# duowuyms/MANSY_ImmersiveVideoStreaming

Hardware: AMD Instinct MI355X
Metric: viewport-trajectories/sec (VP train) (higher is better)
Workload: dtype f32; 1 GPU; VP Transformer train step (fwd+loss+bwd+AdamW), B=4096/GPU synthetic torus-walk trajectories len 21 (hist 10 + cur 1 + pred 10), d=512, 8 heads, 2+2 layers, dropout on, fp32 MFMA, decoder recurrence as two half-batches on two streams; two_stream=True, global_batch=4096, parallelism=dp1

## Files before the change

### include/mansy_hip.h

```cpp
#ifndef MANSY_HIP_H
#define MANSY_HIP_H
#include <stddef.h>
#include <stdint.h>

#ifdef __cplusplus
extern "C" {
#endif

const char* mansy_last_error(void);
int mansy_abi_version(void);

#define MANSY_PREC_F32 0
#define MANSY_PREC_BF16 1
#define MANSY_PREC_BF16X3 3
#define MANSY_PREC_BF16X6 6

typedef int (*mansy_bn_sync_fn)(int which, void* user);

typedef struct mansy_vp_config {
  int B, S, T;
  int d_model, n_head, d_ff;
  int n_enc, n_dec;
  int in_ch;
  int has_bias;
// ... 149 lines not shown
int mansy_identifier_train_step(const float* const* params, float* const* grads, float* flat_p, float* flat_g, float* flat_m,
                                float* flat_v, long long n_flat, const float* obs, const int* idx ,
                                int B, float lr, float weight_decay, int step, float* loss_out, void* workspace, int max_batch,
                                void* xg_ctx ,
                                const float* adam_bias , int precision, void* stream);
int mansy_identifier_relabel(const float* const* params, const float* obs, float* rew, float* id_rew, int B, float lamb,
                             void* workspace, int max_batch, int precision, void* stream);
int mansy_gae_returns(const float* rew, const float* v_s, const float* v_next, const unsigned char* done, int T, int N, double gamma,
                      double gae_lambda, int rew_norm, double* rms, double* scratch, float* returns, float* adv, void* stream);
int mansy_ppo_minibatch_step(const float* const* params, float* const* grads, float* flat_p, float* flat_g, float* flat_m,
                             float* flat_v, long long n_flat, const float* obs_all, const int* idx, const int* act_all,
                             const float* adv_all, const float* logp_old_all, const float* v_old_all, const float* ret_all, int mb,
                             float eps_clip, float vf_coef, float ent_coef, int norm_adv, int value_clip, float dual_clip,
                             float max_grad_norm, float lr, float weight_decay, int step, long long tail_from, int tail_step, float* stats,
                             void* workspace, int max_batch, int chain_in, const int* next_idx, int next_mb, void* xg_ctx, const float* adam_bias,
                             int precision, void* stream);
int mansy_bc_step(const float* const* params, float* const* grads, float* flat_p, float* flat_g, float* flat_m, float* flat_v,
                  long long n_flat, long long n_update, const float* obs, const int* act, int B, float ent_coef, float lr,
                  float weight_decay, int step, float* stats, void* workspace, int max_batch, int precision, void* stream);

#define MANSY_CLIP_SCRATCH_DOUBLES 64
int mansy_clip_grad_adam(float* flat_p, float* flat_g, float* flat_m, float* flat_v, long long n_flat, float max_grad_norm, float lr,
                         float weight_decay, int step, long long tail_from, int tail_step, double* scratch, int have_sumsq,
                         const float* adam_bias , void* stream);

int mansy_ppo_dp_tail(const float* const* params, float* flat_p, float* flat_g, float* flat_m, float* flat_v, long long n_flat,
                      float max_grad_norm, float lr, float weight_decay, int step, double* scratch, int have_sumsq, const float* obs_all,
                      const float* adv_all, const int* next_idx, int next_mb, float* next_flat_g, const float* adam_bias , void* workspace,
                      int max_batch, int precision, void* stream);

typedef struct mansy_comm_id { unsigned char bytes[128]; } mansy_comm_id;
int mansy_comm_unique_id(mansy_comm_id* out);
int mansy_comm_create(const mansy_comm_id* id, int world, int rank, void** comm_out);
int mansy_comm_destroy(void* comm);
int mansy_allreduce_avg_f32(void* comm, float* buf , long long n, void* stream);
int mansy_allreduce_sum_f64(void* comm, double* buf , long long n, void* stream);
int mansy_allgather_f64(void* comm, const double* send, double* recv , long long n_per_rank, void* stream);
#define MANSY_SYNC_XG 0x5847
#define MANSY_SYNC_RCCL 0x5243

typedef struct mansy_xg_handle { unsigned char bytes[64]; } mansy_xg_handle;
int mansy_xg_create(long long n_floats, int world, int rank, void** ctx_out);
int mansy_xg_export(void* ctx, mansy_xg_handle* out);
int mansy_xg_import(void* ctx, const mansy_xg_handle* all );
int mansy_xg_set_timeout_ms(void* ctx, double ms);
int mansy_xg_allreduce_avg(void* ctx, float* g , long long n, double* sumsq_parts ,
                           void* stream);
int mansy_xg_slot_ptrs(void* ctx, float** slot0, float** slot1);
int mansy_xg_next_slot(void* ctx);
int mansy_xg_reduce_avg(void* ctx, float* g_out, long long n, double* sumsq_parts , void* stream);
int mansy_xg_status(void* ctx);
int mansy_xg_destroy(void* ctx);

#define MANSY_A2C_OBS_LD 416
#define MANSY_A2C_O_THROUGHPUT 0
#define MANSY_A2C_O_SIZE 8
#define MANSY_A2C_O_REBUFFER 328
#define MANSY_A2C_O_LAST_RATES 329
#define MANSY_A2C_O_PRED_VP 331
int mansy_a2c_num_params(void);
int mansy_a2c_param_info(int idx, char* name, int name_len, long long* numel, int* ndim, long long shape[4]);
size_t mansy_a2c_workspace_bytes(int max_batch);
int mansy_a2c_obs(const float* obs, const float* qoe_parts, const int* actions, const unsigned char* fresh, int n, const int video_rates[5],
                  float* out, void* stream);
int mansy_a2c_forward(const float* const* params, const float* obs, int B, float* probs, float* value, int* act, float* logp, const float* u,
                      uint32_t seed, uint32_t site, int reuse_packed, void* workspace, int max_batch, int precision, void* stream);
int mansy_a2c_minibatch_step(const float* const* params, float* const* grads, float* flat_p, float* flat_g, float* flat_sq, long long n_flat,
                             const float* obs_all, const int* idx, const int* act_all, const float* adv_all, const float* ret_all, int mb,
                             float vf_coef, float ent_coef, float max_grad_norm, float lr, float alpha, float eps, int apply, float* stats,
                             void* workspace, int max_batch, int precision, void* stream);
int mansy_clip_grad_rmsprop(float* flat_p, float* flat_g, float* flat_sq, long long n_flat, float max_grad_norm, float lr, float alpha,
                            float eps, double* scratch, void* stream);

typedef struct mansy_gemm_epilogue {
  const float* bias; int relu; const float* mask_src; int mask_ld; float mask_scale;
  float drop_p; uint32_t drop_seed; uint32_t drop_site; const float* resid; int resid_ld; int accumulate;
  float* a_rowsum; int prec;
  int variant;
} mansy_gemm_epilogue;
#define MANSY_VARIANT_BF16(v) (((v) + 1) & 0xFF)
#define MANSY_VARIANT_NO_WSK 0x100
#define MANSY_VARIANT_NO_WSK_TN 0x200
#define MANSY_VARIANT_NO_PLAIN 0x400
#define MANSY_VARIANT_COL_GROUP(g) ((((g) + 1) & 0xFF) << 16)
int mansy_gemm_f32(const float* A, int lda, int a_kmajor, const float* B, int ldb, int b_kmajor, float* C, int ldc,
                   int M, int N, int K, const mansy_gemm_epilogue* ep, int force_tile, int force_splitk, void* stream);
int mansy_weight_planes(const float* W, int N, int K, uint16_t* out, uint16_t* out_t, long long plane_stride, int n_planes, void* stream);
int mansy_gemm_planes(const float* A, int lda, const float* B, int ldb, int b_kmajor, const uint16_t* planes, long long plane_stride,
                      int planes_ld, float* C, int ldc, int M, int N, int K, const mansy_gemm_epilogue* ep, int force_tile, void* stream);
int mansy_gemm_bf16(const uint16_t* A16, int lda, int a_kmajor, const uint16_t* B16, int ldb, int b_kmajor, float* C, int ldc, uint16_t* C16, int ldc16,
                    int M, int N, int K, const mansy_gemm_epilogue* ep, const uint16_t* resid16, const uint16_t* mask16, int force_tile, int force_splitk, void* stream);
typedef struct mansy_attn_shape {
  int nb, H, Lq, Lk, dh;
  long long q_bs, q_rs, k_bs, k_rs, v_bs, v_rs, o_bs, o_rs;
  float scale;
} mansy_attn_shape;
int mansy_attn_fwd(const float* Q, const float* K, const float* V, float* O, float* P_save, const mansy_attn_shape* s,
                   float drop_p, uint32_t seed, uint32_t site, void* stream);
int mansy_attn_bwd(const float* Q, const float* K, const float* V, const float* P_save, const float* dO, float* dQ,
                   float* dK, float* dV, const mansy_attn_shape* s, float drop_p, uint32_t seed, uint32_t site,
                   int accum_kv, void* stream);
int mansy_layernorm_fwd(const float* a, const float* b, const float* w, const float* bias, float* z_out, float* y,
                        float* mean, float* rstd, int rows, int C, float eps, void* stream);
int mansy_layernorm_bwd(const float* dy, const float* z, const float* mean, const float* rstd, const float* w, float* dz,
                        float* dz_drop, float drop_p, uint32_t seed, uint32_t site, float* dw, float* dbias, int rows,
                        int C, void* stream);

int mansy_layernorm_bwd_parts(int rows);
int mansy_layernorm_bwd_partial(const float* dy, const float* z, const float* mean, const float* rstd, const float* w, float* dz,
                                float* dz_drop, float drop_p, uint32_t seed, uint32_t site, float* partials, int accumulate,
                                int rows, int C, void* stream);
int mansy_ln_partials_reduce(const float* partials, int nparts, int C, float* dw, float* dbias, void* stream);
int mansy_attn_bwd_dq(const float* Q, const float* K, const float* V, const float* P_save, const float* dO, float* dQ,
                      float* dS_out, float* Pk_out, const mansy_attn_shape* s, float drop_p, uint32_t seed, uint32_t site,
                      void* stream);
int mansy_attn_kvgrad(const float* Q_all, long long q_ts, const float* dO_all, long long o_ts, const float* dS_all,
                      const float* Pk_all, float* dK, float* dV, const mansy_attn_shape* s, int T, int accum, void* stream);
int mansy_attn_bwd_selfpull(const float* Q_all, long long q_ts, const float* K, const float* V, const float* P_save,
                            const float* dO_all, long long o_ts, float* dQ, float* dK, float* dV, float* dS_all, float* Pk_all,
                            const mansy_attn_shape* s, int T, int step, float drop_p, uint32_t seed, uint32_t site, void* stream);

int mansy_prof_gemm_enable(int on);
int mansy_prof_gemm_collect(double* total_ms, long long* launches, double* flops);
unsigned long long mansy_prof_launch_count(void);

#ifdef __cplusplus
}
#endif
#endif
```

### mansy_immersivevideostreaming_amd/csrc/gemm_f32.hip

```cpp
#include <vector>
#include "gemm_tile.h"
#include "gemm_wsk.h"

using namespace mansy_gemm;

namespace {

template <int R, bool KMAJ>
struct TileGeom {
  static constexpr int LOADS = R * BK / 4 / NT;
  static constexpr int LDS_FLOATS = KMAJ ? BK * (R + 4) : R * KC_LD;
};

template <int R, bool KMAJ, bool VEC>
__device__ __forceinline__ void load_tile(const float* __restrict__ P, int ld, int row0, int nrows, int k0, int k_end,
                                          float4 (&reg)[TileGeom<R, KMAJ>::LOADS], int tid) {
#pragma unroll
  for (int i = 0; i < TileGeom<R, KMAJ>::LOADS; ++i) {
    const int idx = tid + i * NT;
    int outer, outer_lim, inner0, lim_inner;
    if (!KMAJ) {
      outer = row0 + (idx >> 3); outer_lim = nrows; inner0 = k0 + (idx & 7) * 4; lim_inner = k_end;
    } else {
      constexpr int C4 = R / 4;
// ... 81 lines not shown
  }
  const bool first_n_tile = tile_x == first_tile;
  const int k_begin = blockIdx.z * p.k_per_split;
  const int k_end = min(p.K, k_begin + p.k_per_split);
  const int nk = (k_end - k_begin + BK - 1) / BK;

  f32x16 acc[TM][TN];
#pragma unroll
  for (int i = 0; i < TM; ++i)
#pragma unroll
    for (int j = 0; j < TN; ++j)
#pragma unroll
      for (int e = 0; e < 16; ++e) acc[i][j][e] = 0.f;

  float rowsum = 0.f;
  float4 ra[TileGeom<BM, AK>::LOADS], rb[TileGeom<BN, BKM>::LOADS];
  if (nk > 0) {
    load_tile<BM, AK, VEC>(p.A, p.lda, m0, p.M, k_begin, k_end, ra, tid);
    load_tile<BN, BKM, VEC>(p.B, p.ldb, n0, p.N, k_begin, k_end, rb, tid);
    store_tile<BM, AK>(smem, ra, tid, k_begin, k_end);
    store_tile<BN, BKM>(smem + A_FLOATS, rb, tid, k_begin, k_end);
  }
  __syncthreads();

  for (int kt = 0; kt < nk; ++kt) {
    const int cur = kt & 1;
    if (kt + 1 < nk) {
      const int k0 = k_begin + (kt + 1) * BK;
      load_tile<BM, AK, VEC>(p.A, p.lda, m0, p.M, k0, k_end, ra, tid);
      load_tile<BN, BKM, VEC>(p.B, p.ldb, n0, p.N, k0, k_end, rb, tid);
    }
    const float* a_l = smem + cur * STAGE;
    const float* b_l = a_l + A_FLOATS;
    if (AK && p.ep.a_rowsum && first_n_tile && tid < BM) {
#pragma unroll
      for (int kk = 0; kk < BK; ++kk) rowsum += a_l[kk * (BM + 4) + tid];
    }
#pragma unroll
    for (int chunk = 0; chunk < 2; ++chunk) {
      float af[TM][8], bf[TN][8];
#pragma unroll
      for (int i = 0; i < TM; ++i) read_frag<BM, AK>(a_l, wm * (BM / 2) + i * 32, r, h, chunk, af[i]);
#pragma unroll
      for (int j = 0; j < TN; ++j) read_frag<BN, BKM>(b_l, wn * (BN / 2) + j * 32, r, h, chunk, bf[j]);
#pragma unroll
      for (int kk = 0; kk < 8; ++kk)
#pragma unroll
        for (int i = 0; i < TM; ++i)
#pragma unroll
          for (int j = 0; j < TN; ++j)
            acc[i][j] = __builtin_amdgcn_mfma_f32_32x32x2f32(af[i][kk], bf[j][kk], acc[i][j], 0, 0, 0);
    }
    if (kt + 1 < nk) {
      const int k0n = k_begin + (kt + 1) * BK;
      store_tile<BM, AK>(smem + (cur ^ 1) * STAGE, ra, tid, k0n, k_end);
      store_tile<BN, BKM>(smem + (cur ^ 1) * STAGE + A_FLOATS, rb, tid, k0n, k_end);
    }
    __syncthreads();
  }

  if (AK && p.ep.a_rowsum && first_n_tile && tid < BM && m0 + tid < p.M) atomicAdd(p.ep.a_rowsum + m0 + tid, rowsum);

  gemm_epilogue<BM, BN, 2 * (A_FLOATS + B_FLOATS)>(p, acc, smem, m0, n0, tid, blockIdx.z, p.C);
}

template <int R, bool KMAJ>
__device__ __forceinline__ void dma_offsets(int ld, int row0, int nrows, unsigned (&voff)[R / 32], int tid) {
  const int lane = tid & 63, wave = tid >> 6;
#pragma unroll
  for (int i = 0; i < R / 32; ++i) {
    if (!KMAJ) {
      const int row = i * 32 + wave * 8 + (lane >> 3);
      const int c = (lane & 7) ^ ((row >> 1) & 7);
      voff[i] = (unsigned)((min(row0 + row, nrows - 1) - row0) * ld + c * 4) * 4u;
    } else {
      constexpr int C4 = R / 4;
      const int idx = (i * 4 + wave) * 64 + lane;
      const int kr = idx / C4, c4 = idx % C4;
      voff[i] = (unsigned)(kr * ld + (min(row0 + c4 * 4, nrows - 4) - row0)) * 4u;
    }
  }
}

template <int BM, int BN, bool AK, bool BKM, bool PLAIN = false>
__global__ __launch_bounds__(NT) void gemm_f32_dma_kernel(GemmParams p) {
  constexpr int TM = BM / 64, TN = BN / 64, PA = BM / 32, PB = BN / 32;
  constexpr int A_FLOATS = BM * BK, B_FLOATS = BN * BK, STAGE = A_FLOATS + B_FLOATS;
  constexpr int C_FLOATS = BM * (BN + 4);
  constexpr int SMEM_FLOATS = 2 * STAGE > C_FLOATS ? 2 * STAGE : C_FLOATS;
  __shared__ __attribute__((aligned(1024))) float smem[SMEM_FLOATS];

  const int tid = threadIdx.x;
  const int lane = tid & 63, wave = tid >> 6;
  const int wm = wave >> 1, wn = wave & 1;
  const int r = lane & 31, h = lane >> 5;
  int tile_x, tile_y;
  int split;
  {
    const int per_split = gridDim.x * gridDim.y, nwg = per_split * gridDim.z;
    const int orig = (blockIdx.z * gridDim.y + blockIdx.y) * gridDim.x + blockIdx.x;
    const int q = nwg >> 3, rem = nwg & 7, xcd = orig & 7, local = orig >> 3;
    int t = (xcd < rem ? xcd * (q + 1) : rem * (q + 1) + (xcd - rem) * q) + local;
    if (PLAIN) split = 0;
    else { split = t / per_split; t -= split * per_split; }
    tile_y = t / gridDim.x; tile_x = t - tile_y * gridDim.x;
    if (!PLAIN && p.col_group > 0 && (int)gridDim.x > p.col_group) {
      const int G = p.col_group, gy = gridDim.y, full = ((int)gridDim.x / G) * G;
      if (t < full * gy) { const int g = t / (G * gy), rr = t - g * G * gy; tile_y = rr / G; tile_x = g * G + (rr - tile_y * G); }
      else { const int W = gridDim.x - full, rr = t - full * gy; tile_y = rr / W; tile_x = full + (rr - tile_y * W); }
    }
    if (!PLAIN && BM == 64 && BN == 64 && p.ep.tile_list) { tile_x = p.ep.tile_list[2 * t]; tile_y = p.ep.tile_list[2 * t + 1]; }
  }
  const float* Ap = p.A; const float* Bp = p.B; float* Cp = p.C; float* rowsum_dst = PLAIN ? nullptr : p.ep.a_rowsum;
  if (!PLAIN && p.A2) {
    const int prob = split / p.splits_pp;
    split -= prob * p.splits_pp;
    if (prob) { Ap = p.A2; Bp = p.B2; Cp = p.C2; rowsum_dst = p.a_rowsum2; }
  }
  const int m0 = tile_y * BM, n0 = tile_x * BN;
  const int n_col_tiles = (p.N + BN - 1) / BN;
  int rs_first = 0, rs_cnt = n_col_tiles;
  if (!PLAIN && BM == 64 && p.ep.tile_nrange) {
    const int lo = p.ep.tile_nrange[2 * tile_y], hi = p.ep.tile_nrange[2 * tile_y + 1];
    if (n0 >= hi || n0 + BN <= lo) return;
    rs_first = lo / BN;
    rs_cnt = min(n_col_tiles, (hi + BN - 1) / BN) - rs_first;
  }
  int k_begin = PLAIN ? 0 : split * p.k_per_split;
  int k_end = PLAIN ? p.K : min(p.K, k_begin + p.k_per_split);
  if (!PLAIN && BN == 64 && p.ep.tile_krange) {
    k_begin = max(k_begin, p.ep.tile_krange[2 * tile_x]);
    k_end = min(k_end, p.ep.tile_krange[2 * tile_x + 1]);
  }
  const int nk = max(0, (k_end - k_begin) / BK);

  unsigned voa[PA], vob[PB];
  dma_offsets<BM, AK>(p.lda, m0, p.M, voa, tid);
  dma_offsets<BN, BKM>(p.ldb, n0, p.N, vob, tid);
  const float* sa = AK ? Ap + (long long)k_begin * p.lda + m0 : Ap + (long long)m0 * p.lda + k_begin;
  const float* sb = BKM ? Bp + (long long)k_begin * p.ldb + n0 : Bp + (long long)n0 * p.ldb + k_begin;
  const long long step_a = AK ? (long long)BK * p.lda : BK, step_b = BKM ? (long long)BK * p.ldb : BK;
  const unsigned lds_wave = __builtin_amdgcn_readfirstlane((unsigned)(uintptr_t)smem + (unsigned)wave * 1024u);

  f32x16 acc[TM][TN];
#pragma unroll
  for (int i = 0; i < TM; ++i)
#pragma unroll
    for (int j = 0; j < TN; ++j)
#pragma unroll
      for (int e = 0; e < 16; ++e) acc[i][j][e] = 0.f;

  float rowsum = 0.f;
  if (nk > 0) {
#pragma unroll
    for (int i = 0; i < PA; ++i) glds16(voa[i], sa, lds_wave + i * 4096u);
#pragma unroll
    for (int i = 0; i < PB; ++i) glds16(vob[i], sb, lds_wave + A_FLOATS * 4u + i * 4096u);
  }
  for (int kt = 0; kt < nk; ++kt) {
    const int cur = kt & 1;
    asm volatile("s_waitcnt vmcnt(0)" ::: "memory");
    __builtin_amdgcn_s_barrier();
    asm volatile("" ::: "memory");
    sa += step_a; sb += step_b;
    const unsigned lds_next = lds_wave + (unsigned)(cur ^ 1) * (STAGE * 4u);
    if (kt + 1 < nk) {
#pragma unroll
      for (int i = 0; i < PA; ++i) glds16(voa[i], sa, lds_next + i * 4096u);
#pragma unroll
      for (int i = 0; i < PB; ++i) glds16(vob[i], sb, lds_next + A_FLOATS * 4u + i * 4096u);
    }
    const float* a_l = smem + cur * STAGE;
    const float* b_l = a_l + A_FLOATS;
    if (AK && rowsum_dst && tid < BM) {
      for (int kk = tile_x - rs_first; kk < BK; kk += rs_cnt) rowsum += a_l[kk * BM + tid];
    }
#pragma unroll
    for (int chunk = 0; chunk < 2; ++chunk) {
      float af[TM][8], bf[TN][8];
#pragma unroll
      for (int i = 0; i < TM; ++i) read_frag_dma<BM, AK>(a_l, wm * (BM / 2) + i * 32, r, h, chunk, af[i]);
#pragma unroll
      for (int j = 0; j < TN; ++j) read_frag_dma<BN, BKM>(b_l, wn * (BN / 2) + j * 32, r, h, chunk, bf[j]);
#pragma unroll
      for (int kk = 0; kk < 8; ++kk)
#pragma unroll
        for (int i = 0; i < TM; ++i)
#pragma unroll
          for (int j = 0; j < TN; ++j)
            acc[i][j] = __builtin_amdgcn_mfma_f32_32x32x2f32(af[i][kk], bf[j][kk], acc[i][j], 0, 0, 0);
    }
    asm volatile("s_waitcnt lgkmcnt(0)" ::: "memory");
  }
  __syncthreads();

  if (AK && rowsum_dst && tile_x - rs_first < BK && tid < BM && m0 + tid < p.M) atomicAdd(rowsum_dst + m0 + tid, rowsum);
  if (PLAIN) {
    constexpr int CLD = BN + 4;
#pragma unroll
    for (int i = 0; i < TM; ++i)
#pragma unroll
      for (int j = 0; j < TN; ++j)
#pragma unroll
        for (int e = 0; e < 16; ++e)
          smem[(wm * (BM / 2) + i * 32 + (e & 3) + 8 * (e >> 2) + 4 * h) * CLD + wn * (BN / 2) + j * 32 + r] = acc[i][j][e];
    __syncthreads();
    gemm_epilogue_rows<BM, BN, NT>(p, smem, m0, n0, tid, Cp);
    return;
  }
  gemm_epilogue<BM, BN, SMEM_FLOATS>(p, acc, smem, m0, n0, tid, split, Cp);
}

template <bool AK, bool BKM>
__global__ __launch_bounds__(NT) void gemm_f32_wsk_kernel(GemmParams p) {
  __shared__ __attribute__((aligned(1024))) float smem[WSK_SMEM_FLOATS];
  gemm_f32_wsk_body<AK, BKM>(p, (blockIdx.z * gridDim.y + blockIdx.y) * gridDim.x + blockIdx.x, gridDim.x, gridDim.y, gridDim.z, smem);
}
struct WskGrid { int x, y, z; };
__global__ __launch_bounds__(NT) void gemm_f32_wsk_dual_kernel(GemmParams p1, WskGrid g1, GemmParams p2, WskGrid g2) {
  __shared__ __attribute__((aligned(1024))) float smem[WSK_SMEM_FLOATS];
  const int n1 = g1.x * g1.y * g1.z, orig = blockIdx.x;
  if (orig < n1) gemm_f32_wsk_body<true, true>(p1, orig, g1.x, g1.y, g1.z, smem);
  else gemm_f32_wsk_body<false, true>(p2, orig - n1, g2.x, g2.y, g2.z, smem);
}

template <int BM, int BN>
int launch_dma(const GemmParams& p, int a_kmajor, int b_kmajor, int splits, hipStream_t st) {
  dim3 grid(mansy_ceil_div(p.N, BN), mansy_ceil_div(p.M, BM), splits);
  if (BM == 64 && BN == 64 && p.ep.tile_list) grid = dim3(p.ep.tile_list_n, 1, splits);
  dim3 block(NT);
  const bool plain_form = ((BM == 64 && BN == 64) || (BM == 128 && BN == 64)) && !mansy_var_no_plain(p.ep.variant) && !a_kmajor && splits == 1 && !p.A2 && !p.ep.tile_list && !p.ep.tile_nrange && !p.ep.tile_krange &&
                          !p.ep.a_rowsum && !p.ep.accumulate && p.ep.split_slab == 0 && p.c_vec_ok && !(p.col_group > 0 && (int)grid.x > p.col_group);
  if (plain_form) {
    constexpr int PBM = (BM == 128 && BN == 64) ? 128 : 64;
    if (b_kmajor) MANSY_GEMM_LAUNCH((gemm_f32_dma_kernel<PBM, 64, false, true, true>), grid, block, st, p);
    else MANSY_GEMM_LAUNCH((gemm_f32_dma_kernel<PBM, 64, false, false, true>), grid, block, st, p);
    MANSY_LAUNCH_CHECK();
    return MANSY_OK;
  }
  if (!a_kmajor && !b_kmajor) MANSY_GEMM_LAUNCH((gemm_f32_dma_kernel<BM, BN, false, false>), grid, block, st, p);
  else if (!a_kmajor && b_kmajor) MANSY_GEMM_LAUNCH((gemm_f32_dma_kernel<BM, BN, false, true>), grid, block, st, p);
  else if (a_kmajor && b_kmajor) MANSY_GEMM_LAUNCH((gemm_f32_dma_kernel<BM, BN, true, true>), grid, block, st, p);
  else MANSY_GEMM_LAUNCH((gemm_f32_dma_kernel<BM, BN, true, false>), grid, block, st, p);
  MANSY_LAUNCH_CHECK();
  return MANSY_OK;
}

template <int BM, int BN, bool VEC>
int launch_cfg(const GemmParams& p, int a_kmajor, int b_kmajor, int splits, hipStream_t st) {
  dim3 grid(mansy_ceil_div(p.N, BN), mansy_ceil_div(p.M, BM), splits);
  if (BM == 64 && BN == 64 && p.ep.tile_list) grid = dim3(p.ep.tile_list_n, 1, splits);
  dim3 block(NT);
  if (!a_kmajor && !b_kmajor) MANSY_GEMM_LAUNCH((gemm_f32_kernel<BM, BN, false, false, VEC>), grid, block, st, p);
  else if (!a_kmajor && b_kmajor) MANSY_GEMM_LAUNCH((gemm_f32_kernel<BM, BN, false, true, VEC>), grid, block, st, p);
  else if (a_kmajor && b_kmajor) MANSY_GEMM_LAUNCH((gemm_f32_kernel<BM, BN, true, true, VEC>), grid, block, st, p);
  else MANSY_GEMM_LAUNCH((gemm_f32_kernel<BM, BN, true, false, VEC>), grid, block, st, p);
  MANSY_LAUNCH_CHECK();
  return MANSY_OK;
}

struct ProfState {
  bool on = false;
  std::vector<hipEvent_t> ev;
  size_t used = 0;
  double flops = 0.0;
};
ProfState g_prof;
}
namespace mansy_gemm { hipEvent_t g_ev_start = nullptr, g_ev_stop = nullptr; }

extern "C" int mansy_prof_gemm_enable(int on) {
  g_prof.on = on != 0;
  g_prof.used = 0;
  g_prof.flops = 0.0;
  return MANSY_OK;
}
extern "C" int mansy_prof_gemm_collect(double* total_ms, long long* launches, double* flops) {
  MANSY_HIP_CHECK(hipDeviceSynchronize());
  double ms = 0.0;
  for (size_t i = 0; i + 1 < g_prof.used; i += 2) {
    float t = 0.f;
    MANSY_HIP_CHECK(hipEventElapsedTime(&t, g_prof.ev[i], g_prof.ev[i + 1]));
    ms += t;
  }
  if (total_ms) *total_ms = ms;
  if (launches) *launches = (long long)(g_prof.used / 2);
  if (flops) *flops = g_prof.flops;
  g_prof.used = 0;
  g_prof.flops = 0.0;
  return MANSY_OK;
}

constexpr int WSK_MAX_TILES = 200;
int mansy_gemm_wsk_tn_enabled() { return !mansy_var_no_wsk_tn(0); }

struct WskPending { GemmParams p; int variant; dim3 grid; };
static thread_local bool g_pair_open = false;
static thread_local std::vector<WskPending> g_pair;
static int wsk_launch_one(const WskPending& w, hipStream_t st) {
  if (w.variant == 0) MANSY_GEMM_LAUNCH((gemm_f32_wsk_kernel<false, false>), w.grid, dim3(NT), st, w.p);
  else if (w.variant == 1) MANSY_GEMM_LAUNCH((gemm_f32_wsk_kernel<false, true>), w.grid, dim3(NT), st, w.p);
  else MANSY_GEMM_LAUNCH((gemm_f32_wsk_kernel<true, true>), w.grid, dim3(NT), st, w.p);
  MANSY_LAUNCH_CHECK();
  return MANSY_OK;
}
static int wsk_launch(const GemmParams& p, int variant, dim3 grid, hipStream_t st) {
  WskPending w{p, variant, grid};
  if (g_pair_open) { g_pair.push_back(w); return MANSY_OK; }
  return wsk_launch_one(w, st);
}
int mansy_gemm_capture_begin() {
  if (g_pair_open || g_prof.on) return 0;
  g_pair_open = true; g_pair.clear();
  return 1;
}
int mansy_gemm_capture_end(mansy_gemm::GemmParams* out, int* variant, int* gx, int* gy, int* gz, int max_n) {
  g_pair_open = false;
  std::vector<WskPending> w;
  w.swap(g_pair);
  int n = 0;
  for (const WskPending& x : w) {
    if (n >= max_n) break;
    out[n] = x.p; variant[n] = x.variant; gx[n] = (int)x.grid.x; gy[n] = (int)x.grid.y; gz[n] = (int)x.grid.z; ++n;
  }
  return (int)w.size() <= max_n ? n : -1;
}
// ... 222 lines not shown
```

### mansy_immersivevideostreaming_amd/csrc/mansy_kernels.h

```cpp
#pragma once
#include "mansy_common.h"

struct GemmEpilogue {
  const float* bias = nullptr;
  int relu = 0;
  float relu_slope = 0.f;
  const float* mask_src = nullptr;
  int mask_ld = 0;
  float mask_scale = 1.f;
  float mask_neg = 0.f;
  MansyDrop drop = {0.f, 0u, 0u};
  const float* resid = nullptr;
  int resid_ld = 0;
  int accumulate = 0;
  float* a_rowsum = nullptr;
  long long split_slab = 0;
  const int* tile_krange = nullptr;
  const int* tile_nrange = nullptr;
  float flops_frac = 1.f;
  const int* tile_list = nullptr; int tile_list_n = 0;
  const float* pair_A = nullptr; const float* pair_B = nullptr; float* pair_C = nullptr; float* pair_rowsum = nullptr;
  int prec = 0;
  int variant = 0;
  const float* pre_a = nullptr; const float* pre_b = nullptr; int pre_ld = 0; int pre_col0 = 0;
  const unsigned short* b_planes = nullptr; long long b_plane_stride = 0; int b_planes_ld = 0;
  const unsigned short* a16 = nullptr; int a16_ld = 0;
  const unsigned short* b16 = nullptr; int b16_ld = 0;
  unsigned short* c16 = nullptr; int c16_ld = 0;
  const unsigned short* resid16 = nullptr; const unsigned short* mask16 = nullptr;
};

#ifdef MANSY_LAB
extern int g_mansy_lab_variant;
inline int mansy_variant_of(int v) { return v ? v : g_mansy_lab_variant; }
#else
inline int mansy_variant_of(int v) { return v; }
#endif
inline int mansy_var_bf16(int v) { const int b = mansy_variant_of(v) & 0xFF; return b ? b - 1 : 1; }
inline bool mansy_var_no_wsk(int v) { return (mansy_variant_of(v) & 0x100) != 0; }
inline bool mansy_var_no_wsk_tn(int v) { return (mansy_variant_of(v) & 0x300) != 0; }
inline bool mansy_var_no_plain(int v) { return (mansy_variant_of(v) & 0x400) != 0; }
inline bool mansy_var_no_pair(int v) { return (mansy_variant_of(v) & 0x800) != 0; }
inline int mansy_var_col_group(int v) { const int g = (mansy_variant_of(v) >> 16) & 0xFF; return g ? g - 1 : 12; }

constexpr int MANSY_WPLANE_MAX = 32;
struct MansyWPlaneTab { const float* w[MANSY_WPLANE_MAX]; int N[MANSY_WPLANE_MAX]; int K[MANSY_WPLANE_MAX]; long long off[MANSY_WPLANE_MAX]; int n; };
int mansy_launch_weight_planes(const MansyWPlaneTab& tab, unsigned short* out, unsigned short* out_t, long long plane_stride, int n_planes,
                               hipStream_t st);
int mansy_gemm_effective_splits(int K, int requested);
int mansy_launch_gemm_bf16a(int a_kmajor, int b_kmajor, float* C, int ldc, int M, int N, int K, const GemmEpilogue& ep, int force_tile, int force_splitk,
                            hipStream_t st);
int mansy_launch_gemm_f32(const float* A, int lda, int a_kmajor, const float* B, int ldb, int b_kmajor,
                          float* C, int ldc, int M, int N, int K, const GemmEpilogue& ep, int force_tile,
                          int force_splitk, hipStream_t st);

struct AttnShape {
  int nb;
  int H;
  int Lq, Lk;
  int dh;
  long long q_bs, q_rs, k_bs, k_rs, v_bs, v_rs, o_bs, o_rs;
  float scale;
};
struct AttnImage {
  const float* f = nullptr; unsigned short* s = nullptr;
  int only = 0;
  int kv16 = 0;
};
int mansy_launch_attn_fwd(const float* Q, const float* K, const float* V, float* O, float* P_save,
                          const AttnShape& s, MansyDrop drop, hipStream_t st, AttnImage img = {});
int mansy_launch_attn_bwd(const float* Q, const float* K, const float* V, const float* P_save, const float* dO,
                          float* dQ, float* dK, float* dV, const AttnShape& s, MansyDrop drop, int accum_kv,
                          hipStream_t st, AttnImage img = {});

int mansy_attn_deferred_kv_ok(const AttnShape& s, int T);
int mansy_launch_attn_bwd_dq(const float* Q, const float* K, const float* V, const float* P_save, const float* dO, float* dQ,
                             float* dS_out, float* Pk_out, const AttnShape& s, MansyDrop drop, hipStream_t st, AttnImage img = {});
int mansy_launch_attn_kvgrad(const float* Q_all, long long q_ts, const float* dO_all, long long o_ts, const float* dS_all,
                             const float* Pk_all, float* dK, float* dV, const AttnShape& s, int T, int accum, hipStream_t st, AttnImage img = {});

int mansy_launch_attn_bwd_selfpull(const float* Q_all, long long q_ts, const float* K, const float* V, const float* P_save,
                                   const float* dO_all, long long o_ts, float* dQ, float* dK, float* dV, float* dS_all, float* Pk_all,
                                   const AttnShape& s, int T, int step, MansyDrop drop, hipStream_t st, AttnImage img = {});

int mansy_launch_layernorm_fwd(const float* a, const float* b, const float* w, const float* bias, float* z_out,
                               float* y, float* mean, float* rstd, int rows, int C, float eps, hipStream_t st,
                               unsigned short* y16 = nullptr, const unsigned short* a16 = nullptr);
int mansy_launch_layernorm_bwd(const float* dy, const float* z, const float* mean, const float* rstd, const float* w,
                               float* dz, float* dz_drop, MansyDrop drop, float* dw, float* dbias, int rows, int C,
                               hipStream_t st);

int mansy_ln_bwd_parts(int rows);
bool mansy_ln_bwd_partial_ok(int C);
int mansy_launch_layernorm_bwd_partial(const float* dy, const float* z, const float* mean, const float* rstd, const float* w,
                                       float* dz, float* dz_drop, MansyDrop drop, float* partials, int accumulate, int rows, int C,
                                       hipStream_t st, unsigned short* dz_drop16 = nullptr, const unsigned short* z16 = nullptr);
int mansy_launch_ln_partials_reduce(const float* partials, int nparts, int C, float* dw, float* dbias, hipStream_t st);
constexpr int LN_MULTI_MAX = 64;
struct MansyLnReduce { const float* partials; int nparts; float* dw; float* dbias; };
int mansy_launch_ln_partials_reduce_multi(const MansyLnReduce* sets, int n, int C, hipStream_t st);

struct DistillShape { int B, S, M, C; int sync_world = 1; int (*hook)(int, void*) = nullptr; void* hook_user = nullptr; };
int mansy_bn_sync_invoke(int which, int (*fn)(int, void*), void* user);
int mansy_gemm_wsk_tn_enabled();
int mansy_gemm_pair_begin();
int mansy_gemm_pair_end(hipStream_t st);
constexpr int MANSY_DISTILL_PARTS = 512;
int mansy_launch_distill_fwd(const float* conv, const float* bn_w, const float* bn_b, float* run_mean, float* run_var,
                             long long* num_batches, float* mean_out, float* rstd_out, float* mem, unsigned char* argmax,
                             double* stats_d, const DistillShape& s, int train, float eps, float momentum,
                             hipStream_t st, double* part = nullptr, unsigned short* mem16 = nullptr);
int mansy_launch_distill_bwd(const float* conv, const float* dmem, const unsigned char* argmax, const float* bn_w,
                             const float* bn_b, const float* mean, const float* rstd, float* g_tmp, float* dconv,
                             float* dbn_w, float* dbn_b, double* stats_d, const DistillShape& s, hipStream_t st, double* part = nullptr,
                             unsigned short* dconv16 = nullptr);

struct MansyDecTailFwd {
  const float* a; const float* b; const float* n3_w; const float* n3_b; float* z3; float* y3; float* m3; float* r3;
  const float* dn_w; const float* dn_b; float* dec_out; float* md; float* rd;
  const float* pw; const float* pb; float* tok_next; float* pred_bt; long long pred_stride;
  const float* ew; const float* eb; const float* pe_row; float* emb_next; MansyDrop edrop;
  int rows, C, C6; float eps;
  unsigned short* y3_16 = nullptr; unsigned short* emb_next16 = nullptr;
  const unsigned short* a16 = nullptr; unsigned short* z3_16 = nullptr; int img_only = 0;
// ... 54 lines not shown
```

### mansy_immersivevideostreaming_amd/kernels.py

```python
import ctypes
import math

import torch

from ._lib import (AttnShape, GemmEpilogue, MansyError, check, lib, ptr, stream_ptr,
                   PRECISIONS, get_precision, precision, set_precision)


VARIANT_NO_WSK, VARIANT_NO_WSK_TN, VARIANT_NO_PLAIN = 0x100, 0x200, 0x400


def VARIANT_BF16(v):
    return (v + 1) & 0xFF


def VARIANT_COL_GROUP(g):
    return ((g + 1) & 0xFF) << 16


def _gpu(*ts):
    for t in ts:
        if t is not None and not t.is_cuda:
            raise MansyError('HIP kernels need cuda (ROCm) tensors')


def gemm(A, B, a_kmajor=False, b_kmajor=False, bias=None, relu=False, mask_src=None, mask_scale=1.0, drop=None,
         resid=None, out=None, accumulate=False, force_tile=0, force_splitk=0, a_rowsum=None, prec=None, variant=0):
    _gpu(A, B)
    A, B = A.contiguous(), B.contiguous()
    M, K = (A.shape[1], A.shape[0]) if a_kmajor else A.shape
    N = B.shape[1] if b_kmajor else B.shape[0]
    Kb = B.shape[0] if b_kmajor else B.shape[1]
    assert K == Kb, (A.shape, B.shape)
    if out is None:
        out = torch.zeros(M, N, dtype=torch.float32, device=A.device) if accumulate else \
            torch.empty(M, N, dtype=torch.float32, device=A.device)
    ep = GemmEpilogue()
    ep.bias = ptr(bias).value if bias is not None else None
    ep.relu = int(relu)
    if mask_src is not None:
        ep.mask_src, ep.mask_ld = mask_src.data_ptr(), mask_src.stride(0)
    ep.mask_scale = mask_scale
    if drop is not None:
        ep.drop_p, ep.drop_seed, ep.drop_site = drop
    if resid is not None:
        ep.resid, ep.resid_ld = resid.data_ptr(), resid.stride(0)
    ep.accumulate = int(accumulate)
    if a_rowsum is not None:
        assert a_kmajor and a_rowsum.numel() == M and a_rowsum.dtype == torch.float32
        ep.a_rowsum = a_rowsum.data_ptr()
    if prec is not None:
        ep.prec = int(prec)
    ep.variant = int(variant)
    check(lib().mansy_gemm_f32(ptr(A), A.stride(0), int(a_kmajor), ptr(B), B.stride(0), int(b_kmajor), ptr(out), out.stride(0),
                               M, N, K, ctypes.byref(ep), force_tile, force_splitk, stream_ptr(A.device)), 'mansy_gemm_f32')
    return out


def weight_planes(W, n_planes):
    _gpu(W)
    W = W.contiguous().float()
    N, K = W.shape
    out = torch.empty(n_planes, N, K, dtype=torch.int16, device=W.device)
    out_t = torch.empty(n_planes, K, N, dtype=torch.int16, device=W.device)
    check(lib().mansy_weight_planes(ptr(W), N, K, ptr(out), ptr(out_t), N * K, n_planes, stream_ptr(W.device)), 'mansy_weight_planes')
    return out, out_t


def gemm_planes(A, W, planes, transposed=False, bias=None, relu=False, resid=None, force_tile=0, variant=0):
    _gpu(A, W, planes)
    A, W = A.contiguous(), W.contiguous()
    M = A.shape[0]
    Nw, Kw = W.shape
    N, K = (Kw, Nw) if transposed else (Nw, Kw)
    assert A.shape[1] == K and planes.shape[1:] == (N, K), (A.shape, W.shape, planes.shape)
    out = torch.empty(M, N, dtype=torch.float32, device=A.device)
    ep = GemmEpilogue()
    ep.bias = ptr(bias).value if bias is not None else None
    ep.relu = int(relu)
    ep.mask_scale = 1.0
    if resid is not None:
        ep.resid, ep.resid_ld = resid.data_ptr(), resid.stride(0)
    ep.variant = int(variant)
    check(lib().mansy_gemm_planes(ptr(A), A.stride(0), ptr(W), W.stride(0), int(transposed), ptr(planes), planes.stride(0), planes.stride(1),
                                  ptr(out), out.stride(0), M, N, K, ctypes.byref(ep), force_tile, stream_ptr(A.device)), 'mansy_gemm_planes')
    return out


def _attn_shape(nb, H, Lq, Lk, dh, q, k, v, o):
    s = AttnShape(nb=nb, H=H, Lq=Lq, Lk=Lk, dh=dh, scale=1.0 / math.sqrt(dh))
    s.q_bs, s.q_rs = q
    s.k_bs, s.k_rs = k
# ... 217 lines not shown
```

Measured before the change: 184,900 trajectories/s.

## Software-pipeline LDS fragment reads with MFMA in 128x64 fp32 DMA GEMM

After: 184,600 trajectories/s. Within noise of the previous version (-0.2%).

```diff
diff --git a/include/mansy_hip.h b/include/mansy_hip.h
--- a/include/mansy_hip.h
+++ b/include/mansy_hip.h
@@ -255,6 +255,7 @@
 #define MANSY_VARIANT_NO_WSK 0x100
 #define MANSY_VARIANT_NO_WSK_TN 0x200
 #define MANSY_VARIANT_NO_PLAIN 0x400
+#define MANSY_VARIANT_NO_PIPE 0x2000
 #define MANSY_VARIANT_COL_GROUP(g) ((((g) + 1) & 0xFF) << 16)
 int mansy_gemm_f32(const float* A, int lda, int a_kmajor, const float* B, int ldb, int b_kmajor, float* C, int ldc,
                    int M, int N, int K, const mansy_gemm_epilogue* ep, int force_tile, int force_splitk, void* stream);
diff --git a/mansy_immersivevideostreaming_amd/csrc/gemm_f32.hip b/mansy_immersivevideostreaming_amd/csrc/gemm_f32.hip
--- a/mansy_immersivevideostreaming_amd/csrc/gemm_f32.hip
+++ b/mansy_immersivevideostreaming_amd/csrc/gemm_f32.hip
@@ -187,7 +187,18 @@
   }
 }
 
-template <int BM, int BN, bool AK, bool BKM, bool PLAIN = false>
+template <int TM, int TN, int K0, int K1>
+__device__ __forceinline__ void mfma_steps(const float (&af)[TM][8], const float (&bf)[TN][8], f32x16 (&acc)[TM][TN]) {
+#pragma unroll
+  for (int kk = K0; kk < K1; ++kk)
+#pragma unroll
+    for (int i = 0; i < TM; ++i)
+#pragma unroll
+      for (int j = 0; j < TN; ++j)
+        acc[i][j] = __builtin_amdgcn_mfma_f32_32x32x2f32(af[i][kk], bf[j][kk], acc[i][j], 0, 0, 0);
+}
+
+template <int BM, int BN, bool AK, bool BKM, bool PLAIN = false, bool PIPE = true>
 __global__ __launch_bounds__(NT) void gemm_f32_dma_kernel(GemmParams p) {
   constexpr int TM = BM / 64, TN = BN / 64, PA = BM / 32, PB = BN / 32;
   constexpr int A_FLOATS = BM * BK, B_FLOATS = BN * BK, STAGE = A_FLOATS + B_FLOATS;
@@ -256,46 +267,101 @@
       for (int e = 0; e < 16; ++e) acc[i][j][e] = 0.f;
 
   float rowsum = 0.f;
-  if (nk > 0) {
-#pragma unroll
-    for (int i = 0; i < PA; ++i) glds16(voa[i], sa, lds_wave + i * 4096u);
-#pragma unroll
-    for (int i = 0; i < PB; ++i) glds16(vob[i], sb, lds_wave + A_FLOATS * 4u + i * 4096u);
-  }
-  for (int kt = 0; kt < nk; ++kt) {
-    const int cur = kt & 1;
-    asm volatile("s_waitcnt vmcnt(0)" ::: "memory");
-    __builtin_amdgcn_s_barrier();
-    asm volatile("" ::: "memory");
-    sa += step_a; sb += step_b;
-    const unsigned lds_next = lds_wave + (unsigned)(cur ^ 1) * (STAGE * 4u);
-    if (kt + 1 < nk) {
-#pragma unroll
-      for (int i = 0; i < PA; ++i) glds16(voa[i], sa, lds_next + i * 4096u);
-#pragma unroll
-      for (int i = 0; i < PB; ++i) glds16(vob[i], sb, lds_next + A_FLOATS * 4u + i * 4096u);
-    }
-    const float* a_l = smem + cur * STAGE;
-    const float* b_l = a_l + A_FLOATS;
-    if (AK && rowsum_dst && tid < BM) {
-      for (int kk = tile_x - rs_first; kk < BK; kk += rs_cnt) rowsum += a_l[kk * BM + tid];
-    }
-#pragma unroll
-    for (int chunk = 0; chunk < 2; ++chunk) {
-      float af[TM][8], bf[TN][8];
+  if constexpr (PIPE) {
+    float af0[TM][8], bf0[TN][8], af1[TM][8], bf1[TN][8];
+    auto read_chunk = [&](const float* a_l, int chunk, float (&af)[TM][8], float (&bf)[TN][8]) {
+      const float* b_l = a_l + A_FLOATS;
 #pragma unroll
       for (int i = 0; i < TM; ++i) read_frag_dma<BM, AK>(a_l, wm * (BM / 2) + i * 32, r, h, chunk, af[i]);
 #pragma unroll
       for (int j = 0; j < TN; ++j) read_frag_dma<BN, BKM>(b_l, wn * (BN / 2) + j * 32, r, h, chunk, bf[j]);
-#pragma unroll
-      for (int kk = 0; kk < 8; ++kk)
-#pragma unroll
-        for (int i = 0; i < TM; ++i)
-#pragma unroll
-          for (int j = 0; j < TN; ++j)
-            acc[i][j] = __builtin_amdgcn_mfma_f32_32x32x2f32(af[i][kk], bf[j][kk], acc[i][j], 0, 0, 0);
-    }
-    asm volatile("s_waitcnt lgkmcnt(0)" ::: "memory");
+    };
+    auto dma_tile = [&](unsigned lds_dst) {
+#pragma unroll
+      for (int i = 0; i < PA; ++i) glds16(voa[i], sa, lds_dst + i * 4096u);
+#pragma unroll
+      for (int i = 0; i < PB; ++i) glds16(vob[i], sb, lds_dst + A_FLOATS * 4u + i * 4096u);
+    };
+    if (nk > 0) {
+      dma_tile(lds_wave);
+      if (nk > 1) {
+        sa += step_a; sb += step_b;
+        dma_tile(lds_wave + STAGE * 4u);
+        asm volatile("s_waitcnt vmcnt(%0)" ::"n"(PA + PB) : "memory");
+      } else {
+        asm volatile("s_waitcnt vmcnt(0)" ::: "memory");
+      }
+      __builtin_amdgcn_s_barrier();
+      asm volatile("" ::: "memory");
+      read_chunk(smem, 0, af0, bf0);
+    }
+    for (int kt = 0; kt < nk; ++kt) {
+      const int cur = kt & 1;
+      const float* a_l = smem + cur * STAGE;
+      __builtin_amdgcn_s_waitcnt(0xC07F);
+      read_chunk(a_l, 1, af1, bf1);
+      __builtin_amdgcn_sched_barrier(0);
+      mfma_steps<TM, TN, 0, 8>(af0, bf0, acc);
+      __builtin_amdgcn_sched_barrier(0);
+      if (AK && rowsum_dst && tid < BM) {
+        for (int kk = tile_x - rs_first; kk < BK; kk += rs_cnt) rowsum += a_l[kk * BM + tid];
+      }
+      __builtin_amdgcn_s_waitcnt(0xC07F);
+      asm volatile("s_waitcnt vmcnt(0)" ::: "memory");
+      __builtin_amdgcn_s_barrier();
+      asm volatile("" ::: "memory");
+      __builtin_amdgcn_sched_barrier(0);
+      mfma_steps<TM, TN, 0, 1>(af1, bf1, acc);
+      __builtin_amdgcn_sched_barrier(0);
+      sa += step_a; sb += step_b;
+      if (kt + 2 < nk) dma_tile(lds_wave + (unsigned)cur * (STAGE * 4u));
+      read_chunk(smem + (cur ^ 1) * STAGE, 0, af0, bf0);
+      __builtin_amdgcn_sched_barrier(0);
+      mfma_steps<TM, TN, 1, 8>(af1, bf1, acc);
+      __builtin_amdgcn_sched_barrier(0);
+    }
+  } else {
+    if (nk > 0) {
+#pragma unroll
+      for (int i = 0; i < PA; ++i) glds16(voa[i], sa, lds_wave + i * 4096u);
+#pragma unroll
+      for (int i = 0; i < PB; ++i) glds16(vob[i], sb, lds_wave + A_FLOATS * 4u + i * 4096u);
+    }
+    for (int kt = 0; kt < nk; ++kt) {
+      const int cur = kt & 1;
+      asm volatile("s_waitcnt vmcnt(0)" ::: "memory");
+      __builtin_amdgcn_s_barrier();
+      asm volatile("" ::: "memory");
+      sa += step_a; sb += step_b;
+      const unsigned lds_next = lds_wave + (unsigned)(cur ^ 1) * (STAGE * 4u);
+      if (kt + 1 < nk) {
+#pragma unroll
+        for (int i = 0; i < PA; ++i) glds16(voa[i], sa, lds_next + i * 4096u);
+#pragma unroll
+        for (int i = 0; i < PB; ++i) glds16(vob[i], sb, lds_next + A_FLOATS * 4u + i * 4096u);
+      }
+      const float* a_l = smem + cur * STAGE;
+      const float* b_l = a_l + A_FLOATS;
+      if (AK && rowsum_dst && tid < BM) {
+        for (int kk = tile_x - rs_first; kk < BK; kk += rs_cnt) rowsum += a_l[kk * BM + tid];
+      }
+#pragma unroll
+      for (int chunk = 0; chunk < 2; ++chunk) {
+        float af[TM][8], bf[TN][8];
+#pragma unroll
+        for (int i = 0; i < TM; ++i) read_frag_dma<BM, AK>(a_l, wm * (BM / 2) + i * 32, r, h, chunk, af[i]);
+#pragma unroll
+        for (int j = 0; j < TN; ++j) read_frag_dma<BN, BKM>(b_l, wn * (BN / 2) + j * 32, r, h, chunk, bf[j]);
+#pragma unroll
+        for (int kk = 0; kk < 8; ++kk)
+#pragma unroll
+          for (int i = 0; i < TM; ++i)
+#pragma unroll
+            for (int j = 0; j < TN; ++j)
+              acc[i][j] = __builtin_amdgcn_mfma_f32_32x32x2f32(af[i][kk], bf[j][kk], acc[i][j], 0, 0, 0);
+      }
+      asm volatile("s_waitcnt lgkmcnt(0)" ::: "memory");
+    }
   }
   __syncthreads();
 
@@ -327,6 +393,15 @@
   const int n1 = g1.x * g1.y * g1.z, orig = blockIdx.x;
   if (orig < n1) gemm_f32_wsk_body<true, true>(p1, orig, g1.x, g1.y, g1.z, smem);
   else gemm_f32_wsk_body<false, true>(p2, orig - n1, g2.x, g2.y, g2.z, smem);
+}
+
+constexpr bool dma_pipe_instance(int BM, int BN, bool AK, bool BKM) { return BM == 128 && BN == 64 && !AK; }
+template <int BM, int BN, bool AK, bool BKM, bool PLAIN>
+void launch_dma_order(const GemmParams& p, bool pipe, dim3 grid, dim3 block, hipStream_t st) {
+  if constexpr (dma_pipe_instance(BM, BN, AK, BKM)) {
+    if (pipe) { MANSY_GEMM_LAUNCH((gemm_f32_dma_kernel<BM, BN, AK, BKM, PLAIN, true>), grid, block, st, p); return; }
+  }
+  MANSY_GEMM_LAUNCH((gemm_f32_dma_kernel<BM, BN, AK, BKM, PLAIN, false>), grid, block, st, p);
 }
 
 template <int BM, int BN>
@@ -336,17 +411,18 @@
   dim3 block(NT);
   const bool plain_form = ((BM == 64 && BN == 64) || (BM == 128 && BN == 64)) && !mansy_var_no_plain(p.ep.variant) && !a_kmajor && splits == 1 && !p.A2 && !p.ep.tile_list && !p.ep.tile_nrange && !p.ep.tile_krange &&
                           !p.ep.a_rowsum && !p.ep.accumulate && p.ep.split_slab == 0 && p.c_vec_ok && !(p.col_group > 0 && (int)grid.x > p.col_group);
+  const bool pipe = !mansy_var_no_pipe(p.ep.variant);
   if (plain_form) {
     constexpr int PBM = (BM == 128 && BN == 64) ? 128 : 64;
-    if (b_kmajor) MANSY_GEMM_LAUNCH((gemm_f32_dma_kernel<PBM, 64, false, true, true>), grid, block, st, p);
-    else MANSY_GEMM_LAUNCH((gemm_f32_dma_kernel<PBM, 64, false, false, true>), grid, block, st, p);
+    if (b_kmajor) launch_dma_order<PBM, 64, false, true, true>(p, pipe, grid, block, st);
+    else launch_dma_order<PBM, 64, false, false, true>(p, pipe, grid, block, st);
     MANSY_LAUNCH_CHECK();
     return MANSY_OK;
   }
-  if (!a_kmajor && !b_kmajor) MANSY_GEMM_LAUNCH((gemm_f32_dma_kernel<BM, BN, false, false>), grid, block, st, p);
-  else if (!a_kmajor && b_kmajor) MANSY_GEMM_LAUNCH((gemm_f32_dma_kernel<BM, BN, false, true>), grid, block, st, p);
-  else if (a_kmajor && b_kmajor) MANSY_GEMM_LAUNCH((gemm_f32_dma_kernel<BM, BN, true, true>), grid, block, st, p);
-  else MANSY_GEMM_LAUNCH((gemm_f32_dma_kernel<BM, BN, true, false>), grid, block, st, p);
+  if (!a_kmajor && !b_kmajor) launch_dma_order<BM, BN, false, false, false>(p, pipe, grid, block, st);
+  else if (!a_kmajor && b_kmajor) launch_dma_order<BM, BN, false, true, false>(p, pipe, grid, block, st);
+  else if (a_kmajor && b_kmajor) launch_dma_order<BM, BN, true, true, false>(p, pipe, grid, block, st);
+  else launch_dma_order<BM, BN, true, false, false>(p, pipe, grid, block, st);
   MANSY_LAUNCH_CHECK();
   return MANSY_OK;
 }
diff --git a/mansy_immersivevideostreaming_amd/csrc/mansy_kernels.h b/mansy_immersivevideostreaming_amd/csrc/mansy_kernels.h
--- a/mansy_immersivevideostreaming_amd/csrc/mansy_kernels.h
+++ b/mansy_immersivevideostreaming_amd/csrc/mansy_kernels.h
@@ -40,6 +40,7 @@
 inline bool mansy_var_no_wsk(int v) { return (mansy_variant_of(v) & 0x100) != 0; }
 inline bool mansy_var_no_wsk_tn(int v) { return (mansy_variant_of(v) & 0x300) != 0; }
 inline bool mansy_var_no_plain(int v) { return (mansy_variant_of(v) & 0x400) != 0; }
+inline bool mansy_var_no_pipe(int v) { return (mansy_variant_of(v) & 0x2000) != 0; }
 inline bool mansy_var_no_pair(int v) { return (mansy_variant_of(v) & 0x800) != 0; }
 inline int mansy_var_col_group(int v) { const int g = (mansy_variant_of(v) >> 16) & 0xFF; return g ? g - 1 : 12; }
 
diff --git a/mansy_immersivevideostreaming_amd/kernels.py b/mansy_immersivevideostreaming_amd/kernels.py
--- a/mansy_immersivevideostreaming_amd/kernels.py
+++ b/mansy_immersivevideostreaming_amd/kernels.py
@@ -8,6 +8,7 @@
 
 
 VARIANT_NO_WSK, VARIANT_NO_WSK_TN, VARIANT_NO_PLAIN = 0x100, 0x200, 0x400
+VARIANT_NO_PIPE = 0x2000
 
 
 def VARIANT_BF16(v):
```
